# kupc25648/MOP-truss-MARL

Measured on AMD Instinct MI355X. Metric: env steps/sec (batched FEM solves) at 4096 envs, higher is better.
Workload: dtype f64; 1 GPU; synthetic random-geometry 2-row trusses, 32 nodes / 80 elements / 60 DOF, FEM-only env.step (action decode + FP64 assembly/solve + stresses + point), no agent; envs_per_gpu=4096, global_envs=4096, nodes=32, elements=80, ndof=60, half_bandwidth=7, lanes_per_env=16, rows_per_lane=1, parallelism=env-batch sharded over 1 GPU(s), no data-path collective

## Files before the change

mop-truss-marl_amd/csrc/truss_body.h:

```cpp
#pragma once
#include <stdint.h>
#include <math.h>

#ifndef TB_SCHED_FENCE
#define TB_SCHED_FENCE()
#endif
#ifndef TRUSS_HD
#error "define TRUSS_HD (e.g. __device__ __forceinline__) before including truss_body.h"
#endif

#define TF_TOP 1
#define TF_RESX 2
#define TF_RESY 4
#define TF_LOAD_BRIDGE 8
#define TF_LOAD_ROOF 16

#define TB_NO_DECODE 0x1u
#define TB_CLAMP_INPLACE 0x2u
#define TB_EMIT_OBS 0x4u

#if defined(__clang__)
typedef uint32_t tb_u4 __attribute__((ext_vector_type(4)));
typedef uint32_t tb_u2 __attribute__((ext_vector_type(2)));
typedef float tb_f4 __attribute__((ext_vector_type(4)));
typedef float tb_f2 __attribute__((ext_vector_type(2)));
typedef double tb_d2 __attribute__((ext_vector_type(2)));
#else
typedef uint32_t tb_u4 __attribute__((vector_size(16)));
typedef uint32_t tb_u2 __attribute__((vector_size(8)));
typedef float tb_f4 __attribute__((vector_size(16)));
typedef float tb_f2 __attribute__((vector_size(8)));
typedef double tb_d2 __attribute__((vector_size(16)));
#endif
TRUSS_HD void tb_ld_row(const double *p, double *dst, int n2) {
  const tb_d2 *q = (const tb_d2 *)__builtin_assume_aligned(p, 16);
  for (int i = 0; i < n2; ++i) {
    tb_d2 v = q[i];
    dst[2 * i] = v[0];
    dst[2 * i + 1] = v[1];
  }
}

struct TopoDev {
  int32_t N, E, NP, ndof, n_pad, n_rest, n_sym_nodes, n_sym_elems, n_sections, has_pairs;
  int32_t nteams, KA, mid, rowsA, rowsB, zlen, dlen, zslot;
  const char *blob;
  int32_t blob_bytes;
  int32_t f_conn;
  int32_t f_pairs;
  int32_t f_nflags;
  int32_t f_dofpos;
  int32_t f_restslot;
  int32_t f_asm;
  int32_t f_diagoff;
  int32_t f_zcode;
  int32_t f_posnode;
  int32_t f_symn;
  int32_t f_syme;
  int32_t f_area;
  int32_t f_isr;
  int32_t f_adj8;
  int32_t f_exs;
  int32_t f_areaf;
  int32_t f_vsf;
  double e_mod, long_stress;
  int32_t o_env0, env_stride;
  int32_t o_kb, o_zs, o_xsol, o_red, o_rbuf, o_par, o_y, o_x, o_tg, o_geo, o_tac, o_sec, o_ev, o_zring, o_mrg;
  int32_t so_q0, so_sr, so_disp, so_mu, so_md, so_comp;
  int32_t emit_ok;
  const char *etab;
  int32_t o_flag;
  int32_t et_xn, et_nxn, et_mat, f_tnxe;
  int32_t nc_xn, nc_nxn, nc_nxe, nc_mat;
  int32_t nxe_cw;
  int32_t b_const;
  int32_t b_erec;
  int32_t b_erec2;
  int32_t b_tc;
  int32_t b_nraw;
  int32_t b_nna, b_nnb, b_nn8;
};

#define TB_TAB(type, base, off) ((const type *)((base) + (off)))

struct StepArgsDev {
  int32_t B;
  uint32_t flags;
  const float *x, *y_in;
  const int32_t *sec_in;
  const float *mu_in, *md_in;
  float *a_geo, *a_topo;
  const uint8_t *coin;
  const float *target;
  const double *env_params;
  float *y_out;
  int32_t *sec_out;
  float *mu_out, *md_out;
  float *disp, *q0, *sr;
  uint8_t *comp;
  float *point, *obj;
  double *disp64, *q064, *energy, *react;
  int32_t *status;
  float *x_n, *A_s, *A_ts, *A_cs, *nxn, *nxe;
};

#define TRUSS_NRED 6

TRUSS_HD float tb_clamp01(float v) { return v > 1.0f ? 1.0f : (v < 0.0f ? 0.0f : v); }

TRUSS_HD float tb_round2(float v) { return rintf(v * 100.0f) / 100.0f; }

template <int G, int WL, int RPL, int EPL, bool EMIT = false>
struct StepLane {
  static constexpr int W = WL * RPL;
  static constexpr int WL_ = WL;
  static constexpr int G_ = G;
  static constexpr bool EMIT_ = EMIT;
  static constexpr int NPL = (2 * EPL + 4) / 5;
  static constexpr int EPB = 64 / G;
  static constexpr int NDEG = 8;
  static constexpr int NT = G / WL;

  int lane, g, gs, team, env, envc;
  double *Kt, *Zt, *ZRt;
  bool active;
  const char *TB;
  char *L;
  double max_def, load_x, load_y;
  float ymax32, dmin32, ymd32, int1, int2;
  int is_roof, heads;
  double ek[EPL], ec[EPL], es[EPL], ei[EPL];
  double R[RPL][W];
  double rhs[RPL];
  double xs[W];
  int bad;
  double p_vol, p_dt, p_en;
  float p_c1, p_c2;

  TRUSS_HD double *kb(const TopoDev &T) { return (double *)(L + T.o_kb); }
  TRUSS_HD double *zs(const TopoDev &T) { return (double *)(L + T.o_zs); }
  TRUSS_HD double *xsol(const TopoDev &T) { return (double *)(L + T.o_xsol); }
  TRUSS_HD double *red(const TopoDev &T) { return (double *)(L + T.o_red); }
  TRUSS_HD double *rbuf(const TopoDev &T) { return (double *)(L + T.o_rbuf); }
  TRUSS_HD double *par(const TopoDev &T) { return (double *)(L + T.o_par); }
  TRUSS_HD float *ysh(const TopoDev &T) { return (float *)(L + T.o_y); }
  TRUSS_HD float *xsh(const TopoDev &T) { return (float *)(L + T.o_x); }
  TRUSS_HD float *tgsh(const TopoDev &T) { return (float *)(L + T.o_tg); }
  TRUSS_HD float *geosh(const TopoDev &T) { return (float *)(L + T.o_geo); }
  TRUSS_HD float *tac(const TopoDev &T) { return (float *)(L + T.o_tac); }
  TRUSS_HD int32_t *secsh(const TopoDev &T) { return (int32_t *)(L + T.o_sec); }
  TRUSS_HD double *evsh(const TopoDev &T) { return (double *)(L + T.o_ev); }
  TRUSS_HD const int16_t *t_conn(const TopoDev &T) const { return TB_TAB(int16_t, TB, T.f_conn); }
  TRUSS_HD const int16_t *t_pairs(const TopoDev &T) const { return TB_TAB(int16_t, TB, T.f_pairs); }
  TRUSS_HD const uint8_t *t_nflags(const TopoDev &T) const { return TB_TAB(uint8_t, TB, T.f_nflags); }
  TRUSS_HD const int16_t *t_dofpos(const TopoDev &T) const { return TB_TAB(int16_t, TB, T.f_dofpos); }
  TRUSS_HD const int16_t *t_restslot(const TopoDev &T) const { return TB_TAB(int16_t, TB, T.f_restslot); }
  TRUSS_HD const int16_t *t_asm(const TopoDev &T) const { return TB_TAB(int16_t, TB, T.f_asm); }
  TRUSS_HD const int16_t *t_diagoff(const TopoDev &T) const { return TB_TAB(int16_t, TB, T.f_diagoff); }
  TRUSS_HD const uint8_t *t_zcode(const TopoDev &T) const { return TB_TAB(uint8_t, TB, T.f_zcode); }
  TRUSS_HD const int16_t *t_posnode(const TopoDev &T) const { return TB_TAB(int16_t, TB, T.f_posnode); }
  TRUSS_HD const int16_t *t_symn(const TopoDev &T) const { return TB_TAB(int16_t, TB, T.f_symn); }
  TRUSS_HD const int16_t *t_syme(const TopoDev &T) const { return TB_TAB(int16_t, TB, T.f_syme); }
  TRUSS_HD const double *t_area(const TopoDev &T) const { return TB_TAB(double, TB, T.f_area); }
  TRUSS_HD const double *t_isr(const TopoDev &T) const { return TB_TAB(double, TB, T.f_isr); }
  TRUSS_HD const int16_t *t_adj8(const TopoDev &T) const { return TB_TAB(int16_t, TB, T.f_adj8); }
  TRUSS_HD const int16_t *t_exs(const TopoDev &T) const { return TB_TAB(int16_t, TB, T.f_exs); }

  TRUSS_HD void init(int lane_, int block, const TopoDev &T, const StepArgsDev &A, char *lds) {
    lane = lane_;
    g = lane % G;
    gs = g % WL;
    team = T.nteams == 2 ? (g / WL) & 1 : 0;
    int grp = lane / G;
    env = block * EPB + grp;
    active = env < A.B;
    envc = active ? env : A.B - 1;
    TB = lds;
    L = lds + T.o_env0 + (size_t)grp * T.env_stride;
    Kt = (double *)(L + T.o_kb) + team * T.rowsA * W;
    Zt = (double *)(L + T.o_zs) + team * T.zlen;
    ZRt = (double *)(L + T.o_zring) + team * W;
    bad = 0;
    p_vol = p_dt = p_en = 0.0;
    p_c1 = p_c2 = 0.0f;
    rs_first_step = 0;
    rs_y_out = A.y_out;
    rs_sec_out = A.sec_out;
    rs_next_geo = rs_next_topo = nullptr;
  }

  static constexpr int BIT = 8;
  static constexpr int BIT_BIG = 20;
  static constexpr int NCAP = (G * ((2 * EPL + 4) / 5) > 64) ? G * ((2 * EPL + 4) / 5) : 64;
  static constexpr int ECAP = (G * EPL > 128) ? G * EPL : 128;
  static constexpr int NIT = (NCAP / 4 + G - 1) / G;
  static constexpr int EIT = (ECAP / 4 + G - 1) / G;
  tb_u4 pg[2 * NIT], pa[3 * NIT];
  int rs_first_step;
  float *rs_y_out;
  int32_t *rs_sec_out;
  const float *rs_next_geo, *rs_next_topo;
  TRUSS_HD void rollout_prefetch(const TopoDev &T, const StepArgsDev &A) {
    if (rs_next_geo) {
      const size_t bn = (size_t)envc * T.N;
      row_load<2 * NIT>(rs_next_geo + bn * 2, 2 * (T.N >> 2), pg);
      row_load<3 * NIT>(rs_next_topo + bn * 3, 3 * (T.N >> 2), pa);
    }
  }
  TRUSS_HD void rollout_stash(const TopoDev &T, const StepArgsDev &A) {
    if (rs_next_geo) {
      row_store<2 * NIT>(geosh(T), 2 * (T.N >> 2), pg);
      row_store<3 * NIT>(tac(T), 3 * (T.N >> 2), pa);
    }
  }

  TRUSS_HD void stage_row_slow(const void *src, void *dst, int nwords) const {
    const uint32_t *s1 = (const uint32_t *)src;
    uint32_t *d1 = (uint32_t *)dst;
    for (int q = g; q < nwords; q += G) d1[q] = s1[q];
  }

  template <int IT>
  TRUSS_HD void row_load(const void *src, int nq, tb_u4 (&v)[IT]) const {
    const tb_u4 *s4 = (const tb_u4 *)src;
#pragma unroll
    for (int i = 0; i < IT; ++i) {
      int q = g + G * i;
      v[i] = s4[q < nq ? q : nq - 1];
    }
  }
  template <int IT>
  TRUSS_HD void row_store(void *dst, int nq, const tb_u4 (&v)[IT]) const {
    tb_u4 *d4 = (tb_u4 *)dst;
#pragma unroll
    for (int i = 0; i < IT; ++i) {
      int q = g + G * i;
      d4[q < nq ? q : nq - 1] = v[i];
    }
  }

  TRUSS_HD void band_clear(const TopoDev &T) {
    tb_u4 *K4 = (tb_u4 *)kb(T);
    const tb_u4 z = {0u, 0u, 0u, 0u};
    const int tot4 = ((T.rowsA + T.rowsB) * W) >> 1;
    for (int i = g; i < tot4; i += G) K4[i] = z;
  }

  template <int BI>
  TRUSS_HD void stage_fast(const TopoDev &T, const StepArgsDev &A, bool decode) {
    const size_t bn = (size_t)envc * T.N, be = (size_t)envc * T.E;
    {
      const int nb = T.blob_bytes >> 4, nn = T.N >> 2, ne = T.E >> 2;
      tb_u4 vb[BI], vy[NIT], vx[NIT], vt[NIT], vs[EIT], vp[1], vg[2 * NIT], va[3 * NIT];
      {
        const tb_u4 *s4 = (const tb_u4 *)T.blob;
#pragma unroll
        for (int i = 0; i < BI; ++i) {
          int q = lane + 64 * i;
          vb[i] = s4[q < nb ? q : nb - 1];
        }
      }
      row_load<NIT>(A.y_in + bn, nn, vy);
      row_load<NIT>(A.x + bn, nn, vx);
      row_load<NIT>(A.target + bn, nn, vt);
      row_load<EIT>(A.sec_in + be, ne, vs);
      row_load<1>(A.env_params + (size_t)envc * 8, 4, vp);
      if (decode) {
        row_load<2 * NIT>(A.a_geo + bn * 2, 2 * nn, vg);
        row_load<3 * NIT>(A.a_topo + bn * 3, 3 * nn, va);
      }
      band_clear(T);
      {
        tb_u4 *d4 = (tb_u4 *)TB;
#pragma unroll
        for (int i = 0; i < BI; ++i) {
          int q = lane + 64 * i;
          d4[q < nb ? q : nb - 1] = vb[i];
        }
      }
      row_store<NIT>(ysh(T), nn, vy);
      row_store<NIT>(xsh(T), nn, vx);
      row_store<NIT>(tgsh(T), nn, vt);
      row_store<EIT>(secsh(T), ne, vs);
      row_store<1>(par(T), 4, vp);
      if (decode) {
        row_store<2 * NIT>(geosh(T), 2 * nn, vg);
        row_store<3 * NIT>(tac(T), 3 * nn, va);
      }
    }
  }

  TRUSS_HD void phase_stage(const TopoDev &T, const StepArgsDev &A) {
    const size_t bn = (size_t)envc * T.N, be = (size_t)envc * T.E;
    const bool decode = !(A.flags & TB_NO_DECODE);
    const bool fast = (T.N & 3) == 0 && (T.E & 3) == 0 && T.N <= NCAP && T.E <= ECAP && T.blob_bytes <= BIT_BIG * 64 * 16;
    heads = A.coin ? (A.coin[envc] != 0) : 0;
    if (rs_first_step != 0) {
      band_clear(T);
      return;
    }
    if (fast) {
      if (T.blob_bytes <= 3 * 64 * 16) stage_fast<3>(T, A, decode);
      else if (T.blob_bytes <= BIT * 64 * 16) stage_fast<BIT>(T, A, decode);
      else stage_fast<BIT_BIG>(T, A, decode);
    } else {
      {
        const tb_u4 *s4 = (const tb_u4 *)T.blob;
        tb_u4 *d4 = (tb_u4 *)TB;
        for (int q = lane; q < (T.blob_bytes >> 4); q += 64) d4[q] = s4[q];
      }
      stage_row_slow(A.y_in + bn, ysh(T), T.N);
      stage_row_slow(A.x + bn, xsh(T), T.N);
      stage_row_slow(A.target + bn, tgsh(T), T.N);
      stage_row_slow(A.sec_in + be, secsh(T), T.E);
      stage_row_slow(A.env_params + (size_t)envc * 8, par(T), 16);
      if (decode) {
        stage_row_slow(A.a_geo + bn * 2, geosh(T), 2 * T.N);
        stage_row_slow(A.a_topo + bn * 3, tac(T), 3 * T.N);
      }
      band_clear(T);
    }
  }

  TRUSS_HD void load_params(const TopoDev &T) {
    const double *P = par(T);
    double y_max = P[0], d_min = P[1];
    max_def = P[2];
    load_x = P[3];
    load_y = P[4];
    int1 = (float)P[5];
    int2 = (float)P[6];
    is_roof = P[7] != 0.0;
    ymax32 = (float)y_max;
    dmin32 = (float)d_min;
    ymd32 = (float)(y_max - d_min);
  }

  TRUSS_HD void move_range(bool top, float y, float yp, float &up, float &dn) const {
    float upt = fabsf(ymax32 - y), dnt = fabsf((y - yp) - dmin32);
    float upb = is_roof ? fabsf((yp - y) - dmin32) : 0.0f, dnb = is_roof ? fabsf(y) : 0.0f;
    up = top ? upt : upb;
    dn = top ? dnt : dnb;
  }

  TRUSS_HD float move_node(float y, float g0, float g1, float mu, float md, bool resy) const {
    bool down = g1 > g0;
    float a = down ? g1 : g0;
    float rng = down ? md : mu;
    float step = (a * rng) * 0.25f;
    y = down ? (y - step) : (y + step);
    y = tb_round2(y);
    return resy ? 0.0f : y;
  }

  struct PairIn {
    int n0, n1, f0, f1;
    float y0, y1, ga0, ga1, gb0, gb1, ta[3], tb[3];
  };
  TRUSS_HD void pair_load(const TopoDev &T, int p, PairIn &q) {
    const float *Y = ysh(T), *GE = geosh(T), *TA = tac(T);
    const int16_t *PR = t_pairs(T);
    const uint8_t *NF = t_nflags(T);
    q.n0 = PR[2 * p];
    q.n1 = PR[2 * p + 1];
    q.y0 = Y[q.n0];
    q.y1 = Y[q.n1];
    q.f0 = NF[q.n0];
    q.f1 = NF[q.n1];
    q.ga0 = GE[2 * q.n0];
    q.ga1 = GE[2 * q.n0 + 1];
    q.gb0 = GE[2 * q.n1];
    q.gb1 = GE[2 * q.n1 + 1];
#pragma unroll
    for (int j = 0; j < 3; ++j) {
      q.ta[j] = TA[3 * q.n0 + j];
      q.tb[j] = TA[3 * q.n1 + j];
    }
  }
  TRUSS_HD void pair_decode(const TopoDev &T, const StepArgsDev &A, PairIn &q, bool real) {
    const size_t bn = (size_t)envc * T.N;
    float *Y = ysh(T), *TA = tac(T);
    const int n0 = q.n0, n1 = q.n1;
    const bool top0 = q.f0 & TF_TOP, top1 = q.f1 & TF_TOP;
    const float ga0 = tb_clamp01(q.ga0), ga1 = tb_clamp01(q.ga1), gb0 = tb_clamp01(q.gb0), gb1 = tb_clamp01(q.gb1);
#pragma unroll
    for (int j = 0; j < 3; ++j) {
      q.ta[j] = tb_clamp01(q.ta[j]);
      q.tb[j] = tb_clamp01(q.tb[j]);
      TA[3 * n0 + j] = q.ta[j];
      TA[3 * n1 + j] = q.tb[j];
    }
    if ((A.flags & TB_CLAMP_INPLACE) && active && real) {
      A.a_geo[(bn + n0) * 2 + 0] = ga0;
      A.a_geo[(bn + n0) * 2 + 1] = ga1;
      A.a_geo[(bn + n1) * 2 + 0] = gb0;
      A.a_geo[(bn + n1) * 2 + 1] = gb1;
#pragma unroll
      for (int j = 0; j < 3; ++j) {
        A.a_topo[(bn + n0) * 3 + j] = q.ta[j];
        A.a_topo[(bn + n1) * 3 + j] = q.tb[j];
      }
    }
    float mu0, md0, mu1, md1;
    if (A.mu_in) {
      mu0 = A.mu_in[bn + n0];
      md0 = A.md_in[bn + n0];
      mu1 = A.mu_in[bn + n1];
      md1 = A.md_in[bn + n1];
    } else {
      move_range(top0, q.y0, q.y1, mu0, md0);
      move_range(top1, q.y1, q.y0, mu1, md1);
    }
    float a = move_node(q.y0, ga0, ga1, mu0, md0, q.f0 & TF_RESY);
    float b = move_node(q.y1, gb0, gb1, mu1, md1, q.f1 & TF_RESY);
    const bool c1 = a < 0.0f;
    a = c1 ? (top0 ? dmin32 : 0.0f) : a;
    b = (c1 && top0) ? 0.0f : b;
    const bool c2 = b < 0.0f;
    b = c2 ? (top1 ? dmin32 : 0.0f) : b;
    a = (c2 && top1) ? 0.0f : a;
    const bool c3 = a > ymax32;
    a = c3 ? (top0 ? ymax32 : ymd32) : a;
    b = (c3 && !top0) ? ymax32 : b;
    const bool c4 = b > ymax32;
    b = c4 ? (top1 ? ymax32 : ymd32) : b;
    a = (c4 && !top1) ? ymax32 : a;
    a = (top0 && fabsf(a - b) < dmin32) ? b + dmin32 : a;
    b = (top1 && fabsf(b - a) < dmin32) ? a + dmin32 : b;
    if (real) {
      Y[n0] = a;
      Y[n1] = b;
    }
  }
  TRUSS_HD void phase_decode(const TopoDev &T, const StepArgsDev &A) {
    load_params(T);
    if (A.flags & TB_NO_DECODE) return;
    constexpr int PPL = (NPL + 1) / 2;
    PairIn q[PPL];
#pragma unroll
    for (int i = 0; i < PPL; ++i) {
      const int p = g + G * i;
      pair_load(T, p < T.NP ? p : T.NP - 1, q[i]);
    }
#pragma unroll
    for (int i = 0; i < PPL; ++i) pair_decode(T, A, q[i], g + G * i < T.NP);
    for (int p = g + G * PPL; p < T.NP; p += G) {
      PairIn r;
      pair_load(T, p, r);
      pair_decode(T, A, r, true);
    }
  }

  TRUSS_HD void phase_sym_nodes(const TopoDev &T) {
    float *Y = ysh(T);
    const int16_t *SN = t_symn(T);
    for (int i = g; i < T.n_sym_nodes; i += G) {
      int dst = SN[2 * i], src = SN[2 * i + 1];
      float v = heads ? Y[src] : Y[dst];
      Y[dst] = v;
      Y[src] = v;
    }
  }

  TRUSS_HD void phase_sizing(const TopoDev &T, const StepArgsDev &A) {
    if (A.flags & TB_NO_DECODE) return;
    const float *TA = tac(T);
    int32_t *S = secsh(T);
    const int16_t *CN = t_conn(T);
    int n0[EPL], n1[EPL], sc[EPL];
    float a0[EPL][3], a1[EPL][3];
#pragma unroll
    for (int i = 0; i < EPL; ++i) {
      const int e = g + G * i;
      const int ee = e < T.E ? e : T.E - 1;
      const uint32_t c = *(const uint32_t *)(CN + 2 * ee);
      n0[i] = (int)(int16_t)(c & 0xffffu);
      n1[i] = (int)(int16_t)(c >> 16);
      sc[i] = S[ee];
    }
#pragma unroll
    for (int i = 0; i < EPL; ++i) {
#pragma unroll
      for (int j = 0; j < 3; ++j) {
        a0[i][j] = TA[n0[i] * 3 + j];
        a1[i][j] = TA[n1[i] * 3 + j];
      }
    }
#pragma unroll
    for (int i = 0; i < EPL; ++i) {
      const float p0 = a0[i][0] + a1[i][0], p1 = a0[i][1] + a1[i][1], p2 = a0[i][2] + a1[i][2];
      int am = 0;
      float best = p0;
      if (p1 > best) { am = 1; best = p1; }
      if (p2 > best) { am = 2; }
      const int s = sc[i];
      const int sdn = s > 0 ? s - 1 : 0, sup = s < T.n_sections - 1 ? s + 1 : T.n_sections - 1;
      sc[i] = am == 0 ? sdn : (am == 1 ? sup : s);
    }
#pragma unroll
    for (int i = 0; i < EPL; ++i) {
      const int e = g + G * i;
      if (e < T.E) S[e] = sc[i];
    }
  }

  TRUSS_HD void phase_sym_elems(const TopoDev &T) {
    int32_t *S = secsh(T);
    const int16_t *SE = t_syme(T);
    for (int i = g; i < T.n_sym_elems; i += G) {
      int a = SE[2 * i], b = SE[2 * i + 1];
      int m = S[a] < S[b] ? S[a] : S[b];
      S[a] = m;
      S[b] = m;
    }
  }

  TRUSS_HD double load_at(const TopoDev &T, int r) const {
    if (r < 0 || r >= T.ndof) return 0.0;
    int nd = t_posnode(T)[r];
    if (nd < 0) return 0.0;
    int fl = t_nflags(T)[nd >> 1] & (is_roof ? TF_LOAD_ROOF : TF_LOAD_BRIDGE);
    if (!fl) return 0.0;
    return (nd & 1) ? load_y : load_x;
  }
  TRUSS_HD int orig_pos(const TopoDev &T, int tm, int p) const { return tm ? T.ndof - 1 - p : p; }
  TRUSS_HD double team_load(const TopoDev &T, int tm, int p) const {
    if (T.nteams == 1) return load_at(T, p);
    if (tm == 0) return p < T.ndof - T.KA ? load_at(T, p) : 0.0;
    return p < T.KA ? load_at(T, T.ndof - 1 - p) : 0.0;
  }

  TRUSS_HD void phase_elements(const TopoDev &T, const StepArgsDev &A) {
    const float *Y = ysh(T), *X = xsh(T);
    const int32_t *S = secsh(T);
    const int16_t *CN = t_conn(T);
    const double *AR = t_area(T), *ISR = t_isr(T);
    double *K = kb(T);
    double kcc[EPL], kcs[EPL], kss[EPL];
#pragma unroll
    for (int i = 0; i < EPL; ++i) {
      const int e = g + G * i;
      const int ee = e < T.E ? e : T.E - 1;
      const int n0 = CN[2 * ee], n1 = CN[2 * ee + 1];
      const int sc = S[ee];
      const double dx = (double)X[n1] - (double)X[n0];
      const double dy = (double)Y[n1] - (double)Y[n0];
      const double l2 = dx * dx + dy * dy;
      const double rl = tb_rsqrt(l2);
      const double len = l2 * rl;
      const double c = dx * rl, s = dy * rl;
      const double Aa = AR[sc];
      const double k = (T.e_mod * Aa) * rl;
      ek[i] = k;
      ec[i] = c;
      es[i] = s;
      ei[i] = ISR[sc];
      if constexpr (EMIT) el[i] = (float)len;
      if (e < T.E) p_vol += (double)(float)(Aa * len);
      const double kc = k * c, ks = k * s;
      kcc[i] = kc * c;
      kcs[i] = kc * s;
      kss[i] = ks * s;
    }
    const int16_t *AC = t_asm(T);
    double *EV = evsh(T);
    if (g == 0) EV[3 * T.E] = EV[3 * T.E + 1] = EV[3 * T.E + 2] = 0.0;
#pragma unroll
    for (int i = 0; i < EPL; ++i) {
      const int e = g + G * i;
      const int ee = e < T.E ? e : T.E - 1;
      EV[3 * ee + 0] = kcc[i];
      EV[3 * ee + 1] = kcs[i];
      EV[3 * ee + 2] = kss[i];
      const int16_t *code = AC + ee * 4;
      K[code[0]] = -kcc[i];
      K[code[1]] = -kss[i];
      K[code[2]] = -kcs[i];
      K[code[3]] = -kcs[i];
    }
  }

  TRUSS_HD void phase_assemble_nodes(const TopoDev &T) {
    const double *EV = evsh(T);
    const int16_t *AD = t_adj8(T), *DO = t_diagoff(T);
    double *K = kb(T);
    static_assert(NDEG == 8, "adjacency rows are read as one 16-byte unit");
    tb_u4 adj[NPL];
    int dof[NPL][3];
    double cc[NPL], cs[NPL], ss[NPL];
#pragma unroll
    for (int i = 0; i < NPL; ++i) {
      const int n0 = g + G * i, n = n0 < T.N ? n0 : T.N - 1;
      adj[i] = *(const tb_u4 *)(AD + n * NDEG);
      dof[i][0] = DO[3 * n];
      dof[i][1] = DO[3 * n + 1];
      dof[i][2] = DO[3 * n + 2];
      cc[i] = cs[i] = ss[i] = 0.0;
    }
#pragma unroll
    for (int h = 0; h < 2; ++h) {
      double ev[NPL][4][3];
#pragma unroll
      for (int i = 0; i < NPL; ++i)
#pragma unroll
        for (int a = 0; a < 4; ++a) {
          const uint32_t w = adj[i][2 * h + (a >> 1)];
          const int e = (a & 1) ? (int)(w >> 16) : (int)(w & 0xffffu);
          ev[i][a][0] = EV[3 * e + 0];
          ev[i][a][1] = EV[3 * e + 1];
          ev[i][a][2] = EV[3 * e + 2];
        }
#pragma unroll
      for (int i = 0; i < NPL; ++i)
#pragma unroll
        for (int a = 0; a < 4; ++a) {
          cc[i] += ev[i][a][0];
          cs[i] += ev[i][a][1];
          ss[i] += ev[i][a][2];
        }
    }
#pragma unroll
    for (int i = 0; i < NPL; ++i) {
      K[dof[i][0]] = cc[i];
      K[dof[i][1]] = ss[i];
      K[dof[i][2]] = cs[i];
    }
    for (int n = g + G * NPL; n < T.N; n += G) {
      double c2 = 0.0, s2 = 0.0, x2 = 0.0;
#pragma unroll
      for (int a = 0; a < NDEG; ++a) {
        const int e = AD[n * NDEG + a];
        c2 += EV[3 * e + 0];
        x2 += EV[3 * e + 1];
        s2 += EV[3 * e + 2];
      }
      K[DO[3 * n]] = c2;
      K[DO[3 * n + 1]] = s2;
      K[DO[3 * n + 2]] = x2;
    }
    const int idA = T.nteams == 1 ? T.ndof : T.ndof - T.KA;
    for (int r = idA + g; r < T.rowsA; r += G) K[r * W + r % W] = 1.0;
    for (int r = T.KA + T.mid + g; r < T.rowsB; r += G) K[(T.rowsA + r) * W + r % W] = 1.0;
  }

  TRUSS_HD void solver_scratch_init(const TopoDev &T) {
    double *Z = zs(T);
    const uint8_t *ZC = t_zcode(T);
    const int lbit = is_roof ? 4 : 2;
    {
      const int zt = T.zlen * T.nteams;
      constexpr int ZIT = 6;
#pragma unroll
      for (int i = 0; i < ZIT; ++i) {
        const int r0 = g + G * i, r = r0 < zt ? r0 : zt - 1;
        const int c = ZC[r];
        Z[r] = (c & lbit) ? ((c & 1) ? load_y : load_x) : 0.0;
      }
      for (int r = g + G * ZIT; r < zt; r += G) {
        const int c = ZC[r];
        Z[r] = (c & lbit) ? ((c & 1) ? load_y : load_x) : 0.0;
      }
    }
    tb_d2 *X2 = (tb_d2 *)__builtin_assume_aligned(xsol(T), 16);
    const tb_d2 z2 = {0.0, 0.0};
    for (int r = g; r < (T.zslot + 2) / 2; r += G) X2[r] = z2;
    double *RB = rbuf(T);
    for (int i = g; i < T.n_rest; i += G) RB[i] = 0.0;
  }

  TRUSS_HD void solver_init(const TopoDev &T) {
#pragma unroll
    for (int s = 0; s < RPL; ++s) {
      int r = gs + WL * s;
#pragma unroll
      for (int c = 0; c < W; ++c) R[s][c] = (c <= r) ? Kt[r * W + c] : Kt[c * W + r];
      rhs[s] = Zt[r];
    }
#pragma unroll
    for (int j = 0; j < W; ++j) xs[j] = 0.0;
  }

  double zkeep[RPL];
  TRUSS_HD void pivot_write(const TopoDev &T, int k, int kk) {
#pragma unroll
    for (int s = 0; s < RPL; ++s) Kt[k * W + gs + WL * s] = R[s][kk];
    bx = rhs[kk / WL];
  }
  TRUSS_HD void factor_z_store(const TopoDev &T, int kb, int c, int cnt) {
#pragma unroll
    for (int s = 0; s < RPL; ++s) {
      const int off = (gs + WL * s - c + W) % W;
      double *zp = off < cnt ? Zt + kb + off : ZRt + gs;
      *zp = zkeep[s];
    }
  }

  TRUSS_HD void pivot_update(const TopoDev &T, int k, int kk) {
    double col[W];
    {
      const double *Kn = Kt + (k + W) * W;
#pragma unroll
      for (int s = 0; s < RPL; ++s) ecol[s] = Kn[gs + WL * s];
    }
#pragma unroll
    for (int i = 0; i < W / 2; ++i) {
      tb_d2 v = ((const tb_d2 *)__builtin_assume_aligned(Kt + k * W, 16))[i];
      col[2 * i] = v[0];
      col[2 * i + 1] = v[1];
    }
    const double zk = tb_team_bcast(*this, kk % WL);
    if (gs == kk % WL) zkeep[kk / WL] = bx;
    const double d = col[kk];
    const double inv = tb_rcp(d);
#pragma unroll
    for (int s = 0; s < RPL; ++s) {
      double l = R[s][kk] * inv;
#pragma unroll
      for (int j = 0; j < W; ++j)
        if (j != kk) R[s][j] = fma(-l, col[j], R[s][j]);
      rhs[s] = fma(-l, zk, rhs[s]);
    }
#pragma unroll
    for (int s = 0; s < RPL; ++s) R[s][kk] = ecol[s];
    if (gs == kk % WL) {
      const int sp = kk / WL;
#pragma unroll
      for (int j = 0; j < W; ++j)
        if (j != kk) R[sp][j] = fr[sp][j];
      rhs[sp] = frhs[sp];
    }
  }
// ... 1069 lines not shown
```

mop-truss-marl_amd/csrc/truss_hip.hip:

```cpp
#include <hip/hip_runtime.h>

#include <atomic>
#include <cstdint>
#include <cstdio>
#include <cstring>
#include <type_traits>

#include "../../include/truss_mi355.h"

#pragma clang fp contract(off)

#define TRUSS_HD __device__ __forceinline__
#define TRUSS_UNROLL _Pragma("unroll")
#define TB_SCHED_FENCE() __builtin_amdgcn_sched_barrier(0)
#define TB_STREAM_STORE(p, v) __builtin_nontemporal_store((v), (p))
#ifdef TRUSS_OBS_STORE_NT
#define TB_OBS_STORE(p, v) __builtin_nontemporal_store((v), (p))
#else
#define TB_OBS_STORE(p, v) (*(p) = (v))
#endif

__device__ __forceinline__ void tb_lds_add(double *p, double v) { unsafeAtomicAdd(p, v); }

template <int WL, int SRC>
// ... 115 lines not shown
  if constexpr (LN::EMIT_) return *((const __attribute__((address_space(3))) int *)(ln.TB + T.o_flag) + 1) != 0;
  return false;
}

#include "truss_body.h"

typedef __attribute__((address_space(3))) int tb_lds_word;
__device__ __forceinline__ tb_lds_word *tb_flag_ptr(char *lds, int o_flag) { return (tb_lds_word *)(lds + o_flag); }
__device__ __forceinline__ void tb_publish(char *lds, int o_flag, int k) {
  __builtin_amdgcn_wave_barrier();
#ifdef TRUSS_FLAG_RELAXED
  __builtin_amdgcn_fence(__ATOMIC_RELEASE, "wavefront");
  if (threadIdx.x == 0) __hip_atomic_store(tb_flag_ptr(lds, o_flag), k, __ATOMIC_RELAXED, __HIP_MEMORY_SCOPE_WORKGROUP);
#else
  if (threadIdx.x == 0) __hip_atomic_store(tb_flag_ptr(lds, o_flag), k, __ATOMIC_RELEASE, __HIP_MEMORY_SCOPE_WORKGROUP);
#endif
}
#ifndef TB_AWAIT_SPINS
#define TB_AWAIT_SPINS (1 << 22)
#endif
__device__ __forceinline__ bool tb_await(char *lds, int o_flag, int k) {
  for (int spin = 0; spin < TB_AWAIT_SPINS; ++spin) {
    const int v = __hip_atomic_load(tb_flag_ptr(lds, o_flag), __ATOMIC_ACQUIRE, __HIP_MEMORY_SCOPE_WORKGROUP);
    if (__builtin_amdgcn_readfirstlane(v) >= k) return true;
    __builtin_amdgcn_s_sleep(1);
  }
  return false;
}

template <class LN>
__device__ __forceinline__ void tb_obs_timeout(LN &ln, char *lds, int o_flag, int32_t *status) {
  if ((threadIdx.x & 63) == 0) *(tb_flag_ptr(lds, o_flag) + 1) = 1;
  if (ln.g == 0 && ln.active && status) atomicOr(&status[ln.env], TRUSS_STATUS_OBS_TIMEOUT);
}

template <int G, int WL, int RPL, int EPL, bool EMIT>
__global__ __launch_bounds__(EMIT ? 128 : 64) void truss_step_kernel(const TopoDev T, const StepArgsDev A) {
  extern __shared__ __attribute__((aligned(16))) char smem[];
  StepLane<G, WL, RPL, EPL, EMIT> ln;
  ln.init(threadIdx.x & 63, blockIdx.x, T, A, smem);
  constexpr int W_ = StepLane<G, WL, RPL, EPL, EMIT>::W;
  constexpr bool EMIT_ = EMIT;
  if constexpr (EMIT) {
    if (threadIdx.x == 0) {
      *tb_flag_ptr(smem, T.o_flag) = 0;
      *(tb_flag_ptr(smem, T.o_flag) + 1) = 0;
    }
    __syncthreads();
    if (threadIdx.x >= 64) {
#define SPH(call) \
  ln.call;        \
  __builtin_amdgcn_fence(__ATOMIC_RELEASE, "wavefront"); \
  __builtin_amdgcn_wave_barrier();                        \
  __builtin_amdgcn_fence(__ATOMIC_ACQUIRE, "wavefront")
#ifdef TRUSS_STAMPS
#define SST(i)                                                                                        \
  do {                                                                                                \
    __builtin_amdgcn_sched_barrier(0);                                                                \
    if (threadIdx.x == 64 && blockIdx.x == gridDim.x / 2) g_truss_stamps[i] = clock64();              \
    if (threadIdx.x == 64 && ((i) == 20 || (i) == 26) && blockIdx.x < 4096)                           \
      g_truss_span[blockIdx.x][(i) == 20 ? 4 : 5] = wall_clock64();                                   \
    __builtin_amdgcn_sched_barrier(0);                                                                \
  } while (0)
#else
#define SST(i)
#endif
      ln.emit_tables_load(T);
      __builtin_amdgcn_s_waitcnt(0);
      bool ok = tb_await(smem, T.o_flag, 1);
      if (ok) {
        SST(20);
        TRUSS_STREAM_SEG1(SPH, T, A)
        SST(21);
        ok = tb_await(smem, T.o_flag, 2);
      }
      if (ok) {
        SST(22);
        TRUSS_STREAM_SEG2(SPH, T, A)
        SST(23);
        ok = tb_await(smem, T.o_flag, 3);
      }
      if (ok) {
        SST(24);
        TRUSS_STREAM_SEG3(SPH, T, A)
        SST(25);
      } else {
        tb_obs_timeout(ln, smem, T.o_flag, A.status);
      }
#ifdef TRUSS_STAMPS
      __builtin_amdgcn_s_waitcnt(0);
      SST(26);
#endif
#undef SST
#undef SPH
      return;
    }
  }
#define TB_WAVE_SYNC()                                    \
  do {                                                    \
    __builtin_amdgcn_fence(__ATOMIC_RELEASE, "wavefront"); \
    __builtin_amdgcn_wave_barrier();                      \
    __builtin_amdgcn_fence(__ATOMIC_ACQUIRE, "wavefront"); \
  } while (0)
#define PH(call) \
  ln.call;       \
  TB_WAVE_SYNC()
#define PH_NS(call) ln.call
#define BAR() TB_WAVE_SYNC()
#ifdef TRUSS_FAULT_DROP_PUBLISH3
#define EMIT_POINT(k) do { if ((k) != 3) tb_publish(smem, T.o_flag, k); } while (0)
#else
#define EMIT_POINT(k) tb_publish(smem, T.o_flag, k)
#endif
  TRUSS_STEP_SCHEDULE(PH, PH_NS, BAR, T, A)
#undef PH
#undef PH_NS
#undef BAR
#undef EMIT_POINT
#undef TB_WAVE_SYNC
}

struct RolloutDev {
  TopoDev T;
  StepArgsDev A;
  int32_t n_steps, n_sets;
  size_t gstride, tstride;
};
template <int G, int WL, int RPL, int EPL>
__global__ __launch_bounds__(64) void truss_rollout_kernel(const RolloutDev P_) {
  extern __shared__ __attribute__((aligned(16))) char smem[];
  constexpr int W_ = StepLane<G, WL, RPL, EPL, false>::W;
  constexpr bool EMIT_ = false;
#define TB_WAVE_SYNC()                                    \
  do {                                                    \
    __builtin_amdgcn_fence(__ATOMIC_RELEASE, "wavefront"); \
    __builtin_amdgcn_wave_barrier();                      \
    __builtin_amdgcn_fence(__ATOMIC_ACQUIRE, "wavefront"); \
  } while (0)
#define PH(call) \
  ln.call;       \
  TB_WAVE_SYNC()
#define PH_NS(call) ln.call
#define BAR() TB_WAVE_SYNC()
#define EMIT_POINT(k) (void)0
  const int n_steps = P_.n_steps;
  for (int s = 0; s < n_steps; ++s) {
    typedef const char __attribute__((address_space(4))) *tb_kernarg_ptr;
    tb_kernarg_ptr ka = (tb_kernarg_ptr)__builtin_amdgcn_kernarg_segment_ptr();
    asm volatile("" : "+s"(ka));
    const RolloutDev &P = *(const RolloutDev *)ka;
    const TopoDev &T = P.T;
    const StepArgsDev &A = P.A;
    StepLane<G, WL, RPL, EPL, false> ln;
    ln.init(threadIdx.x, blockIdx.x, T, A, smem);
    const int nset = (s + 1) % P.n_sets;
    ln.rs_first_step = s;
    ln.rs_y_out = (s & 1) ? (float *)A.y_in : A.y_out;
    ln.rs_sec_out = (s & 1) ? (int32_t *)A.sec_in : A.sec_out;
    ln.rs_next_geo = s + 1 < n_steps ? A.a_geo + (size_t)nset * P.gstride : nullptr;
    ln.rs_next_topo = s + 1 < n_steps ? A.a_topo + (size_t)nset * P.tstride : nullptr;
    TRUSS_STEP_SCHEDULE(PH, PH_NS, BAR, T, A)
    TB_WAVE_SYNC();
  }
#undef PH
#undef PH_NS
#undef BAR
#undef EMIT_POINT
#undef TB_WAVE_SYNC
}

__global__ __launch_bounds__(64) void truss_obs_kernel(const TopoDev T, const ObsArgsDev A) {
  extern __shared__ __attribute__((aligned(16))) char smem[];
  ObsLane ln;
  ln.init(threadIdx.x, blockIdx.x, blockIdx.y, T, A, smem);
#define PH(call) \
  ln.call;       \
  __syncthreads()
#define PH_NS(call) ln.call
  const int r0_tile = ln.role == 1 ? ((int)blockIdx.y - 1) * A.tile_rows : 0;
  TRUSS_OBS_SCHEDULE(PH, PH_NS, T, A, r0_tile)
#undef PH
#undef PH_NS
}

__global__ __launch_bounds__(64) void truss_front_kernel(const truss_front_args_t A) {
  __shared__ double px[64], py[64], pc1[64], pc2[64];
  __shared__ double sx[64], sy[64], sd[64], scr[64];
  __shared__ int sidx[64], keep[64];
  __shared__ double ax[64], ay[64];
  const int b = blockIdx.x, i = threadIdx.x, P = A.max_points;
  int n = A.n_points[b];
  n = n < 0 ? 0 : (n > P ? P : n);
  const bool have = i < n;
  const double *row = A.points + ((size_t)b * P + (have ? i : 0)) * 4;
  const double x = row[0], y = row[1], c1 = row[2], c2 = row[3];
  px[i] = x; py[i] = y; pc1[i] = c1; pc2[i] = c2;
  __syncthreads();
  const bool feas = have && !(c1 > 1.0 || c2 > 1.0);
  bool dom = false, dup = false;
  for (int j = 0; j < n; ++j) {
    const bool fj = !(pc1[j] > 1.0 || pc2[j] > 1.0);
    dom |= fj && px[j] < x && py[j] < y;
    dup |= fj && j < i && px[j] == x && py[j] == y && pc1[j] == c1 && pc2[j] == c2;
  }
  const bool fr = feas && !dom && !dup;
  const double cx = fmin(x, 1.0), cy = fmin(y, 1.0);
  keep[i] = fr ? 1 : 0;
  __syncthreads();
  int rank = 0, arank = 0;
  for (int j = 0; j < n; ++j) {
    rank += keep[j] && (px[j] < x || (px[j] == x && (py[j] < y || (py[j] == y && j < i))));
    const double cxj = fmin(px[j], 1.0);
    arank += (cxj < cx || (cxj == cx && j < i));
  }
  __syncthreads();
  const unsigned long long fmask = __ballot(fr);
  int nf = __popcll(fmask);
  if (fr) { sx[rank] = x; sy[rank] = y; sidx[rank] = i; }
  if (have) { ax[arank] = cx; ay[arank] = cy; }
  __syncthreads();
  if (i + 1 < nf) {
    const double dx = sx[i] - sx[i + 1], dy = sy[i] - sy[i + 1];
    sd[i] = sqrt(dx * dx + dy * dy);
  }
  __syncthreads();
  if (i < nf) scr[i] = nf == 1 ? 0.0 : (i == 0 ? sd[0] : (i == nf - 1 ? sd[nf - 2] : sd[i - 1] + sd[i]));
  __syncthreads();
  bool kp = i < nf;
  if ((A.flags & TRUSS_FRONT_TRUNCATE) && nf > A.max_front) {
    if (i > 0 && i < nf - 1) {
      int cr = 0;
      for (int j = 1; j < nf - 1; ++j) cr += (scr[j] > scr[i] || (scr[j] == scr[i] && j < i));
      kp = cr < A.max_front - 2;
    }
  }
  const unsigned long long kmask = __ballot(kp);
  const int pos = __popcll(kmask & ((1ull << i) - 1ull));
  const int nk = __popcll(kmask);
  const double kx = i < nf ? sx[i] : 0.0, ky = i < nf ? sy[i] : 0.0;
  const int kid = i < nf ? sidx[i] : -1;
  __syncthreads();
  if (kp) { sx[pos] = kx; sy[pos] = ky; keep[pos] = kid; }
  nf = nk;
  __syncthreads();
  if (i + 1 < nf) {
    const double dx = sx[i] - sx[i + 1], dy = sy[i] - sy[i + 1];
    sd[i] = sqrt(dx * dx + dy * dy);
  }
  if (A.front_idx && i < P) A.front_idx[(size_t)b * P + i] = i < nf ? keep[i] : -1;
  __syncthreads();
  if (i != 0) return;
  if (A.n_front) A.n_front[b] = nf;
  const double rx = A.ref_points ? A.ref_points[2 * b] : 1.0, ry = A.ref_points ? A.ref_points[2 * b + 1] : 1.0;
  if (A.metrics) {
    double maxd = 0.0, disd = 1.0, sumd = 0.0, stdcd = 1.0, pn = 0.0;
    if (nf >= 2) {
      maxd = sd[0];
      for (int k = 0; k < nf - 1; ++k) { maxd = sd[k] > maxd ? sd[k] : maxd; sumd += sd[k]; }
      double acc = 0.0;
      const double ctr = maxd / (nf - 1);
      for (int k = 0; k < nf - 1; ++k) acc += (sd[k] - ctr) * (sd[k] - ctr);
      disd = sqrt(acc / (nf - 1));
    }
    if (nf > 3) {
      double s = 0.0, mx = 0.0;
      for (int k = 1; k < nf - 1; ++k) {
        const double cd = fabs(sx[k - 1] - sx[k + 1]) + fabs(sy[k - 1] - sy[k + 1]);
        scr[k] = cd; s += cd; mx = cd > mx ? cd : mx;
      }
      if (s != 0.0) {
        const int m = nf - 2;
        double mean = 0.0;
        for (int k = 1; k < nf - 1; ++k) { scr[k] = scr[k] / mx; mean += scr[k]; }
        mean /= m;
        double var = 0.0, p10 = 0.0;
        for (int k = 1; k < nf - 1; ++k) {
          const double v = scr[k], d = v - mean;
          var += d * d;
          const double v2 = v * v, v4 = v2 * v2;
          p10 += v4 * v4 * v2;
        }
        stdcd = sqrt(var / m);
        pn = pow(p10, 0.1);
      }
    }
    double *M = A.metrics + (size_t)b * 5;
    M[0] = maxd; M[1] = disd; M[2] = pn; M[3] = sumd; M[4] = stdcd;
  }
  if (A.hv_front) {
    double hv = 0.0;
    if (nf > 0 && !(nf == 1 && sx[0] == 1.0 && sy[0] == 1.0)) {
      double area = 0.0, runmin = 1.0, minx = sx[0], miny = sy[0];
      for (int k = 0; k < nf; ++k) {
        const double cxk = fmin(sx[k], 1.0), cyk = fmin(sy[k], 1.0);
        runmin = cyk < runmin ? cyk : runmin;
        const double nx = k + 1 < nf ? fmin(sx[k + 1], 1.0) : 1.0;
        area += (nx - cxk) * (1.0 - runmin);
        minx = sx[k] < minx ? sx[k] : minx;
        miny = sy[k] < miny ? sy[k] : miny;
      }
      hv = area - ((1.0 - rx) * (1.0 - minx) + (1.0 - ry) * (1.0 - miny) - (1.0 - rx) * (1.0 - ry));
    }
    A.hv_front[b] = hv;
  }
  if (A.hv_all) {
    double hv = 0.0;
    if (n > 0 && !(n == 1 && px[0] == 1.0 && py[0] == 1.0)) {
// ... 535 lines not shown
```

Measured before the change: 224.3 million env-steps/s.

## Batch element loads, stage coin flag in LDS, and hoist mu/md range loads

```diff
diff --git a/mop-truss-marl_amd/csrc/truss_body.h b/mop-truss-marl_amd/csrc/truss_body.h
--- a/mop-truss-marl_amd/csrc/truss_body.h
+++ b/mop-truss-marl_amd/csrc/truss_body.h
@@ -128,7 +128,7 @@
   char *L;
   double max_def, load_x, load_y;
   float ymax32, dmin32, ymd32, int1, int2;
-  int is_roof, heads;
+  int is_roof;
   double ek[EPL], ec[EPL], es[EPL], ei[EPL];
   double R[RPL][W];
   double rhs[RPL];
@@ -149,6 +149,10 @@
   TRUSS_HD float *geosh(const TopoDev &T) { return (float *)(L + T.o_geo); }
   TRUSS_HD float *tac(const TopoDev &T) { return (float *)(L + T.o_tac); }
   TRUSS_HD int32_t *secsh(const TopoDev &T) { return (int32_t *)(L + T.o_sec); }
+  TRUSS_HD int32_t *coinsh(const TopoDev &T) { return (int32_t *)(L + T.env_stride - 4); }
+  TRUSS_HD static bool coin_used(const TopoDev &T, const StepArgsDev &A) {
+    return T.n_sym_nodes > 0 && !(A.flags & TB_NO_DECODE) && A.coin;
+  }
   TRUSS_HD double *evsh(const TopoDev &T) { return (double *)(L + T.o_ev); }
   TRUSS_HD const int16_t *t_conn(const TopoDev &T) const { return TB_TAB(int16_t, TB, T.f_conn); }
   TRUSS_HD const int16_t *t_pairs(const TopoDev &T) const { return TB_TAB(int16_t, TB, T.f_pairs); }
@@ -269,6 +273,9 @@
         row_load<2 * NIT>(A.a_geo + bn * 2, 2 * nn, vg);
         row_load<3 * NIT>(A.a_topo + bn * 3, 3 * nn, va);
       }
+      const bool coin = coin_used(T, A);
+      int cb = 0;
+      if (coin) cb = A.coin[envc];
       band_clear(T);
       {
         tb_u4 *d4 = (tb_u4 *)TB;
@@ -287,6 +294,7 @@
         row_store<2 * NIT>(geosh(T), 2 * nn, vg);
         row_store<3 * NIT>(tac(T), 3 * nn, va);
       }
+      if (coin) *coinsh(T) = cb;
     }
   }
 
@@ -294,7 +302,6 @@
     const size_t bn = (size_t)envc * T.N, be = (size_t)envc * T.E;
     const bool decode = !(A.flags & TB_NO_DECODE);
     const bool fast = (T.N & 3) == 0 && (T.E & 3) == 0 && T.N <= NCAP && T.E <= ECAP && T.blob_bytes <= BIT_BIG * 64 * 16;
-    heads = A.coin ? (A.coin[envc] != 0) : 0;
     if (rs_first_step != 0) {
       band_clear(T);
       return;
@@ -304,6 +311,9 @@
       else if (T.blob_bytes <= BIT * 64 * 16) stage_fast<BIT>(T, A, decode);
       else stage_fast<BIT_BIG>(T, A, decode);
     } else {
+      const bool coin = coin_used(T, A);
+      int cb = 0;
+      if (coin) cb = A.coin[envc];
       {
         const tb_u4 *s4 = (const tb_u4 *)T.blob;
         tb_u4 *d4 = (tb_u4 *)TB;
@@ -319,6 +329,7 @@
         stage_row_slow(A.a_topo + bn * 3, tac(T), 3 * T.N);
       }
       band_clear(T);
+      if (coin) *coinsh(T) = cb;
     }
   }
 
@@ -356,6 +367,7 @@
   struct PairIn {
     int n0, n1, f0, f1;
     float y0, y1, ga0, ga1, gb0, gb1, ta[3], tb[3];
+    float mu0, md0, mu1, md1;
   };
   TRUSS_HD void pair_load(const TopoDev &T, int p, PairIn &q) {
     const float *Y = ysh(T), *GE = geosh(T), *TA = tac(T);
@@ -377,6 +389,13 @@
       q.tb[j] = TA[3 * q.n1 + j];
     }
   }
+  TRUSS_HD void pair_ranges_load(const TopoDev &T, const StepArgsDev &A, PairIn &q) const {
+    const size_t bn = (size_t)envc * T.N;
+    q.mu0 = A.mu_in[bn + q.n0];
+    q.md0 = A.md_in[bn + q.n0];
+    q.mu1 = A.mu_in[bn + q.n1];
+    q.md1 = A.md_in[bn + q.n1];
+  }
   TRUSS_HD void pair_decode(const TopoDev &T, const StepArgsDev &A, PairIn &q, bool real) {
     const size_t bn = (size_t)envc * T.N;
     float *Y = ysh(T), *TA = tac(T);
@@ -403,10 +422,10 @@
     }
     float mu0, md0, mu1, md1;
     if (A.mu_in) {
-      mu0 = A.mu_in[bn + n0];
-      md0 = A.md_in[bn + n0];
-      mu1 = A.mu_in[bn + n1];
-      md1 = A.md_in[bn + n1];
+      mu0 = q.mu0;
+      md0 = q.md0;
+      mu1 = q.mu1;
+      md1 = q.md1;
     } else {
       move_range(top0, q.y0, q.y1, mu0, md0);
       move_range(top1, q.y1, q.y0, mu1, md1);
@@ -442,11 +461,16 @@
       const int p = g + G * i;
       pair_load(T, p < T.NP ? p : T.NP - 1, q[i]);
     }
+    if (A.mu_in) {
+#pragma unroll
+      for (int i = 0; i < PPL; ++i) pair_ranges_load(T, A, q[i]);
+    }
 #pragma unroll
     for (int i = 0; i < PPL; ++i) pair_decode(T, A, q[i], g + G * i < T.NP);
     for (int p = g + G * PPL; p < T.NP; p += G) {
       PairIn r;
       pair_load(T, p, r);
+      if (A.mu_in) pair_ranges_load(T, A, r);
       pair_decode(T, A, r, true);
     }
   }
@@ -454,6 +478,7 @@
   TRUSS_HD void phase_sym_nodes(const TopoDev &T) {
     float *Y = ysh(T);
     const int16_t *SN = t_symn(T);
+    const bool heads = *coinsh(T) != 0;
     for (int i = g; i < T.n_sym_nodes; i += G) {
       int dst = SN[2 * i], src = SN[2 * i + 1];
       float v = heads ? Y[src] : Y[dst];
@@ -530,53 +555,73 @@
     return p < T.KA ? load_at(T, T.ndof - 1 - p) : 0.0;
   }
 
+  static constexpr bool EBATCH = RPL == 1 && W <= 8 && EPL <= 5;
+  static constexpr int ECH = EBATCH ? EPL : 1;
   TRUSS_HD void phase_elements(const TopoDev &T, const StepArgsDev &A) {
     const float *Y = ysh(T), *X = xsh(T);
     const int32_t *S = secsh(T);
     const int16_t *CN = t_conn(T);
     const double *AR = t_area(T), *ISR = t_isr(T);
     double *K = kb(T);
-    double kcc[EPL], kcs[EPL], kss[EPL];
-#pragma unroll
-    for (int i = 0; i < EPL; ++i) {
-      const int e = g + G * i;
-      const int ee = e < T.E ? e : T.E - 1;
-      const int n0 = CN[2 * ee], n1 = CN[2 * ee + 1];
-      const int sc = S[ee];
-      const double dx = (double)X[n1] - (double)X[n0];
-      const double dy = (double)Y[n1] - (double)Y[n0];
-      const double l2 = dx * dx + dy * dy;
-      const double rl = tb_rsqrt(l2);
-      const double len = l2 * rl;
-      const double c = dx * rl, s = dy * rl;
-      const double Aa = AR[sc];
-      const double k = (T.e_mod * Aa) * rl;
-      ek[i] = k;
-      ec[i] = c;
-      es[i] = s;
-      ei[i] = ISR[sc];
-      if constexpr (EMIT) el[i] = (float)len;
-      if (e < T.E) p_vol += (double)(float)(Aa * len);
-      const double kc = k * c, ks = k * s;
-      kcc[i] = kc * c;
-      kcs[i] = kc * s;
-      kss[i] = ks * s;
-    }
     const int16_t *AC = t_asm(T);
     double *EV = evsh(T);
     if (g == 0) EV[3 * T.E] = EV[3 * T.E + 1] = EV[3 * T.E + 2] = 0.0;
 #pragma unroll
-    for (int i = 0; i < EPL; ++i) {
-      const int e = g + G * i;
-      const int ee = e < T.E ? e : T.E - 1;
-      EV[3 * ee + 0] = kcc[i];
-      EV[3 * ee + 1] = kcs[i];
-      EV[3 * ee + 2] = kss[i];
-      const int16_t *code = AC + ee * 4;
-      K[code[0]] = -kcc[i];
-      K[code[1]] = -kss[i];
-      K[code[2]] = -kcs[i];
-      K[code[3]] = -kcs[i];
+    for (int c0 = 0; c0 < EPL; c0 += ECH) {
+      int n0[ECH], n1[ECH], sc[ECH], ev[ECH];
+      tb_u2 code[ECH];
+      float x0[ECH], x1[ECH], y0[ECH], y1[ECH];
+      double Aa[ECH];
+#pragma unroll
+      for (int j = 0; j < ECH; ++j) {
+        const int i = c0 + j < EPL ? c0 + j : EPL - 1;
+        const int e = g + G * i;
+        const int ee = e < T.E ? e : T.E - 1;
+        const uint32_t c = *(const uint32_t *)(CN + 2 * ee);
+        n0[j] = (int)(int16_t)(c & 0xffffu);
+        n1[j] = (int)(int16_t)(c >> 16);
+        sc[j] = S[ee];
+        code[j] = *(const tb_u2 *)(AC + 4 * ee);
+        ev[j] = 3 * ee;
+      }
+#pragma unroll
+      for (int j = 0; j < ECH; ++j) {
+        x0[j] = X[n0[j]];
+        x1[j] = X[n1[j]];
+        y0[j] = Y[n0[j]];
+        y1[j] = Y[n1[j]];
+        Aa[j] = AR[sc[j]];
+      }
+#pragma unroll
+      for (int j = 0; j < ECH; ++j) {
+        const int i = c0 + j;
+        if (i < EPL) {
+          const double dx = (double)x1[j] - (double)x0[j];
+          const double dy = (double)y1[j] - (double)y0[j];
+          const double l2 = dx * dx + dy * dy;
+          const double rl = tb_rsqrt(l2);
+          const double len = l2 * rl;
+          const double c = dx * rl, s = dy * rl;
+          const double k = (T.e_mod * Aa[j]) * rl;
+          ek[i] = k;
+          ec[i] = c;
+          es[i] = s;
+          ei[i] = ISR[sc[j]];
+          if constexpr (EMIT) el[i] = (float)len;
+          const double vol = (double)(float)(Aa[j] * len);
+          if constexpr (EBATCH) p_vol += (g + G * i < T.E) ? vol : 0.0;
+          else if (g + G * i < T.E) p_vol += vol;
+          const double kc = k * c, ks = k * s;
+          const double kcc = kc * c, kcs = kc * s, kss = ks * s;
+          EV[ev[j] + 0] = kcc;
+          EV[ev[j] + 1] = kcs;
+          EV[ev[j] + 2] = kss;
+          K[(int16_t)(code[j][0] & 0xffffu)] = -kcc;
+          K[(int16_t)(code[j][0] >> 16)] = -kss;
+          K[(int16_t)(code[j][1] & 0xffffu)] = -kcs;
+          K[(int16_t)(code[j][1] >> 16)] = -kcs;
+        }
+      }
     }
   }
 
diff --git a/mop-truss-marl_amd/csrc/truss_hip.hip b/mop-truss-marl_amd/csrc/truss_hip.hip
--- a/mop-truss-marl_amd/csrc/truss_hip.hip
+++ b/mop-truss-marl_amd/csrc/truss_hip.hip
@@ -291,7 +291,9 @@
     const TopoDev &T = P.T;
     const StepArgsDev &A = P.A;
     StepLane<G, WL, RPL, EPL, false> ln;
-    ln.init(threadIdx.x, blockIdx.x, T, A, smem);
+    int lane_id = threadIdx.x;
+    asm volatile("" : "+v"(lane_id));
+    ln.init(lane_id, blockIdx.x, T, A, smem);
     const int nset = (s + 1) % P.n_sets;
     ln.rs_first_step = s;
     ln.rs_y_out = (s & 1) ? (float *)A.y_in : A.y_out;
```

Result: faster. 232.5 million env-steps/s, median of 6 (+3.7%).
